# stripe/rainier

Hardware: NVIDIA H100
Metric: leapfrog_steps_x_chains_per_sec (higher is better)
Workload: dtype f64

## Files before the change

rainier_b200/csrc/rn_sampler.cuh:

```cuda
#ifndef RN_SAMPLER_CUH
#define RN_SAMPLER_CUH


#if RN_MASS_MAX >= 1
#define RN_TS_NMASS RN_N
#else
#define RN_TS_NMASS 0
#endif
#if RN_ENABLE_EHMC
#define RN_TS_NSNAP RN_N
#else
#define RN_TS_NSNAP 0
#endif
#ifndef RN_TS_RESTORE
#define RN_TS_RESTORE 0
#endif
#if RN_TS_RESTORE
#define RN_TS_NREST (2 * RN_N + 1)
#else
#define RN_TS_NREST 0
#endif
#define RN_TS_P 0
#define RN_TS_MASS (RN_N + 1)
#define RN_TS_SNAP (RN_TS_MASS + RN_TS_NMASS)
#define RN_TS_STAT (RN_TS_SNAP + RN_TS_NSNAP)
#define RN_TS_HOT (RN_TS_STAT + 5)
#define RN_TS_REST (RN_TS_HOT + 4)
#define RN_TS_DOUBLES (RN_TS_REST + RN_TS_NREST)
#define RN_TS_INTS 10
struct RnTs {
  double* d;
  int* i;
  unsigned bs;
};
#ifdef RN_HOST_EMULATION
static thread_local double rn_ts_mem_d[RN_TS_DOUBLES];
static thread_local int rn_ts_mem_i[RN_TS_INTS];
RN_DEVICE RnTs rn_ts_get() { return RnTs{rn_ts_mem_d, rn_ts_mem_i, 1u}; }
#define RN_STCS(ptr, v) (*(ptr) = (v))
#else
extern __shared__ double rn_ts_mem[];
RN_DEVICE RnTs rn_ts_get() {
  RnTs T;
#ifdef RN_BLOCK_DIM
  T.bs = RN_BLOCK_DIM;
#else
  T.bs = blockDim.x;
#endif
  T.d = rn_ts_mem + threadIdx.x;
  T.i = (int*)(rn_ts_mem + (size_t)RN_TS_DOUBLES * blockDim.x) + threadIdx.x;
  return T;
}
#define RN_STCS(ptr, v) __stcs((ptr), (v))
#endif
#define RN_TSD(slot) T.d[(unsigned)(slot) * T.bs]
#define RN_TSI(slot) T.i[(unsigned)(slot) * T.bs]
#ifndef RN_X_P_REGS
#define RN_X_P_REGS 1
#endif
#ifndef RN_X_NORMALS
#define RN_X_NORMALS 3
#endif
#define RN_Z(i) RN_TSD(RN_TS_P + (i))
#if RN_X_P_REGS
#define RN_P(i) s.p[i]
#else
#define RN_P(i) RN_TSD(RN_TS_P + (i))
#endif
#define RN_MASSD(i) RN_TSD(RN_TS_MASS + (i))
#define RN_SNAP_P(i) RN_TSD(RN_TS_SNAP + (i))
#define RN_ST_E_MEAN RN_TSD(RN_TS_STAT + 0)
#define RN_ST_E_RAW RN_TSD(RN_TS_STAT + 1)
#define RN_ST_TRANS2 RN_TSD(RN_TS_STAT + 2)
#define RN_ST_GRADS RN_TSD(RN_TS_STAT + 3)
#define RN_ST_STEPS RN_TSD(RN_TS_STAT + 4)
#define RN_ST_ITERS RN_TSI(0)
#define RN_ST_ACCEPTED RN_TSI(1)
#define RN_ST_E_N RN_TSI(2)
#define RN_ST_RING_I(r) RN_TSI(3 + (r))
#define RN_ST_RING_FULL(r) RN_TSI(6 + (r))
#define RN_TS_PREV_H RN_TSD(RN_TS_HOT + 2)
#define RN_TS_START_H RN_TSD(RN_TS_HOT + 3)
#define RN_REST_Q(i) RN_TSD(RN_TS_REST + (i))
#define RN_REST_G(i) RN_TSD(RN_TS_REST + RN_N + (i))
#define RN_REST_U RN_TSD(RN_TS_REST + 2 * RN_N)

struct RnIt {
  int grads, steps, err;
};

RN_DEVICE RnRng rn_rng_unpark(const RnTs& T) {
  RnRng r;
  r.seed = rn_d2ll(RN_TSD(RN_TS_HOT + 0));
  r.nng = RN_TSD(RN_TS_HOT + 1);
  r.have = RN_TSI(9);
  return r;
}
RN_DEVICE void rn_rng_park(const RnTs& T, const RnRng& r) {
  RN_TSD(RN_TS_HOT + 0) = rn_ll2d(r.seed);
  RN_TSD(RN_TS_HOT + 1) = r.nng;
  RN_TSI(9) = r.have;
}

RN_DEVICE void rn_ring_add(const RnArgs& A, int c, const RnTs& T, int which, double value) {
  int i = RN_ST_RING_I(which) + 1;
  if (i == A.stats_window) {
    RN_ST_RING_FULL(which) = 1;
    i = 0;
  }
  RN_ST_RING_I(which) = i;
  RN_STCS(&RN_AT(A.st_rings, which * A.stats_window + i, c), value);
}

struct RnPQ {
  double q[RN_N], g[RN_N];
  double U;
#if RN_X_P_REGS
  double p[RN_N];
#endif
};

RN_DEVICE double rn_velocity_i(const RnArgs& A, int c, const RnTs& T, const RnPQ& s, int kind, int i) {
  (void)s;
  (void)T;
  (void)A;
  (void)c;
#if RN_MASS_MAX >= 2
  if (kind == 2) {
    double y = 0.0;
    for (int j = 0; j < RN_N; j++) y += RN_P(j) * RN_AT(A.mass, i * RN_N + j, c);
    return y;
  }
#endif
#if RN_MASS_MAX >= 1
  if (kind == 1) return RN_P(i) * RN_MASSD(i);
#endif
  (void)kind;
  return RN_P(i);
}

RN_DEVICE double rn_energy(const RnArgs& A, int c, const RnTs& T, const RnPQ& s, int kind, double U) {
  double k = 0.0;
#if RN_MASS_MAX >= 2
  if (kind == 2) {
    for (int i = 0; i < RN_N; i++) k += (rn_velocity_i(A, c, T, s, 2, i) * RN_P(i));
    return U + k / 2.0;
  }
#endif
  RN_UNROLL
  for (int i = 0; i < RN_N; i++) k += (rn_velocity_i(A, c, T, s, kind, i) * RN_P(i));
  return U + k / 2.0;
}

RN_DEVICE double rn_log_accept(double deltaH) {
  if (deltaH != deltaH) return -RN_INF;
  return rn_jmin0(-deltaH);
}


RN_DEVICE void rn_update(const RnArgs& A, RnPQ& s, RnIt& S) {
  double dens;
  rn_density(s.q, dens, s.g, A.data, S.err);
  s.U = dens * -1;
  S.grads += 1;
}
RN_DEVICE void rn_full_ps(const RnTs& T, RnPQ& s, double stepSize, RnIt& S) {
  (void)T;
  S.grads += 1;
  RN_UNROLL
  for (int i = 0; i < RN_N; i++) RN_P(i) += stepSize * s.g[i];
}
RN_DEVICE void rn_new_qs(const RnArgs& A, int c, const RnTs& T, int kind, RnPQ& s, double stepSize) {
#if RN_MASS_MAX >= 2
  if (kind == 2) {
    for (int i = 0; i < RN_N; i++) s.q[i] += (stepSize * rn_velocity_i(A, c, T, s, 2, i));
    return;
  }
#endif
  RN_UNROLL
  for (int i = 0; i < RN_N; i++) s.q[i] += (stepSize * rn_velocity_i(A, c, T, s, kind, i));
}
RN_DEVICE void rn_leapfrog(const RnArgs& A, int c, const RnTs& T, int kind, RnPQ& s, int l, double stepSize, RnIt& S) {
  rn_full_ps(T, s, stepSize / 2.0, S);
  for (int i = 0;;) {
    rn_new_qs(A, c, T, kind, s, stepSize);
    rn_update(A, s, S);
    if (++i >= l) break;
    rn_full_ps(T, s, stepSize, S);
  }
  rn_full_ps(T, s, stepSize / 2.0, S);
}
RN_DEVICE void rn_take_steps(const RnArgs& A, int c, const RnTs& T, int kind, RnPQ& s, int l, double stepSize, RnIt& S) {
  rn_ring_add(A, c, T, 0, stepSize);
  rn_leapfrog(A, c, T, kind, s, l, stepSize, S);
  S.steps += l;
}

RN_DEVICE void rn_draw_normals(const RnTs& T, RnRng& rng) {
#if RN_X_NORMALS == 2
  for (int i = 0; i < RN_N; i++) RN_Z(i) = rn_normal(rng);
  return;
#endif
  int i0 = 0;
  if (rng.have) {
    rng.have = 0;
    RN_Z(0) = rng.nng;
    i0 = 1;
  }
  const int npairs = (RN_N - i0 + 1) / 2;
#ifndef RN_X_POLAR2
#define RN_X_POLAR2 1
#endif
#if RN_X_POLAR2
  for (int k = 0; k < npairs;) {
    double a1, a2, b1, b2;
    rn_i64 seed4, seed8;
    rn_polar_attempt2(rng, a1, a2, b1, b2, seed4, seed8);
    const double sa = a1 * a1 + a2 * a2, sb = b1 * b1 + b2 * b2;
    const bool oka = !(sa >= 1 || sa == 0);
    const int kb = k + (oka ? 1 : 0);
    const bool needb = kb < npairs;
    const bool okb = needb && !(sb >= 1 || sb == 0);
    if (oka) {
      RN_Z(i0 + 2 * k) = a1;
      RN_Z(i0 + 2 * k + 1) = a2;
    }
    if (okb) {
      RN_Z(i0 + 2 * kb) = b1;
      RN_Z(i0 + 2 * kb + 1) = b2;
    }
    rng.seed = needb ? seed8 : seed4;
    k = kb + (okb ? 1 : 0);
  }
#else
  for (int k = 0; k < npairs;) {
    double v1, v2;
    rn_polar_attempt(rng, v1, v2);
    const double s = v1 * v1 + v2 * v2;
    if (!(s >= 1 || s == 0)) {
      RN_Z(i0 + 2 * k) = v1;
      RN_Z(i0 + 2 * k + 1) = v2;
      k += 1;
    }
  }
#endif
#if RN_X_NORMALS == 4 && RN_X_SPEC && !defined(RN_FAST_MATH) && !(defined(RN_X_LIBM_PLAIN) && RN_X_LIBM_PLAIN)
#pragma unroll 1
  for (int k = 0; k < npairs; k += 2) {
    const int ia = i0 + 2 * k, ib = i0 + 2 * (k + 1 < npairs ? k + 1 : k);
    const double a1 = RN_Z(ia), a2 = RN_Z(ia + 1), b1 = RN_Z(ib), b2 = RN_Z(ib + 1);
    const double sa = a1 * a1 + a2 * a2, sb = b1 * b1 + b2 * b2;
    bool oka, okb;
    double la = rn_strict_log_try(sa, oka), lb = rn_strict_log_try(sb, okb);
    if (!(oka && okb)) {
      la = rn_strict_log_full(sa);
      lb = rn_strict_log_full(sb);
    }
    const double ma = rn_sqrt_nc(rn_div_nc(-2 * la, sa)), mb = rn_sqrt_nc(rn_div_nc(-2 * lb, sb));
    RN_Z(ia) = a1 * ma;
    if (ia + 1 < RN_N) {
      RN_Z(ia + 1) = a2 * ma;
    } else {
      rng.nng = a2 * ma;
      rng.have = 1;
    }
    RN_Z(ib) = b1 * mb;
    if (ib + 1 < RN_N) {
      RN_Z(ib + 1) = b2 * mb;
    } else {
      rng.nng = b2 * mb;
      rng.have = 1;
    }
  }
  return;
#endif
#if RN_X_NORMALS == 1
#pragma unroll 1
#elif RN_X_NORMALS == 3
#pragma unroll 2
#endif
  for (int k = 0; k < npairs; k++) {
    const int i = i0 + 2 * k;
    const double v1 = RN_Z(i), v2 = RN_Z(i + 1);
    const double s = v1 * v1 + v2 * v2;
    const double multiplier = rn_polar_multiplier(s);
    RN_Z(i) = v1 * multiplier;
    if (i + 1 < RN_N) {
      RN_Z(i + 1) = v2 * multiplier;
    } else {
      rng.nng = v2 * multiplier;
      rng.have = 1;
    }
  }
}

RN_DEVICE void rn_initialize_ps(const RnArgs& A, int c, const RnTs& T, RnPQ& s, int kind, RnRng& rng) {
  (void)A;
  (void)c;
  (void)kind;
  (void)s;
  rn_draw_normals(T, rng);
#if RN_X_P_REGS
  RN_UNROLL
  for (int i = 0; i < RN_N; i++) s.p[i] = RN_Z(i);
#endif
#if RN_MASS_MAX >= 2
  if (kind == 2) {
    int i = RN_N - 1;
    int m = ((i + 1) * (i + 2)) / 2 - 1;
    while (i >= 0) {
      int j = RN_N - 1;
      double dot = 0.0;
      while (j > i) {
        dot += RN_Z(j) * RN_AT(A.chol, m, c);
        j -= 1;
        m -= 1;
      }
      RN_Z(i) = (RN_Z(i) - dot) / RN_AT(A.chol, m, c);
      i -= 1;
      m -= 1;
    }
#if RN_X_P_REGS
    for (int k = 0; k < RN_N; k++) s.p[k] = RN_Z(k);
#endif
    return;
  }
#endif
#if RN_MASS_MAX >= 1
  if (kind == 1) {
    RN_UNROLL
    for (int i = 0; i < RN_N; i++) RN_P(i) = RN_P(i) / sqrt(RN_MASSD(i));
    return;
  }
#endif
}

RN_DEVICE void rn_load_mass(const RnArgs& A, int c, const RnTs& T, int kind) {
  (void)A;
  (void)c;
  (void)T;
  (void)kind;
#if RN_MASS_MAX >= 1
  if (kind == 1) {
    RN_UNROLL
    for (int i = 0; i < RN_N; i++) RN_MASSD(i) = RN_AT(A.mass, i, c);
  }
#endif
}

RN_DEVICE void rn_load_stats(const RnArgs& A, int c, const RnTs& T) {
  RN_ST_GRADS = rn_ll2d(A.st_grads[c]);
  RN_ST_STEPS = rn_ll2d(A.st_steps[c]);
  RN_ST_ITERS = A.st_iters[c];
  RN_ST_ACCEPTED = A.st_accepted[c];
  RN_ST_E_MEAN = RN_AT(A.st_energy, 0, c);
  RN_ST_E_RAW = RN_AT(A.st_energy, 1, c);
  RN_ST_TRANS2 = RN_AT(A.st_energy, 2, c);
  RN_ST_E_N = A.st_energy_n[c];
  for (int r = 0; r < 3; r++) {
    RN_ST_RING_I(r) = RN_AT(A.st_ring_i, r, c);
    RN_ST_RING_FULL(r) = RN_AT(A.st_ring_full, r, c);
  }
}
RN_DEVICE void rn_store_stats(const RnArgs& A, int c, const RnTs& T, int err) {
  A.st_grads[c] = rn_d2ll(RN_ST_GRADS);
  A.st_steps[c] = rn_d2ll(RN_ST_STEPS);
  A.st_iters[c] = RN_ST_ITERS;
  A.st_accepted[c] = RN_ST_ACCEPTED;
  if (err) A.st_err[c] |= err;
  RN_AT(A.st_energy, 0, c) = RN_ST_E_MEAN;
  RN_AT(A.st_energy, 1, c) = RN_ST_E_RAW;
  RN_AT(A.st_energy, 2, c) = RN_ST_TRANS2;
  A.st_energy_n[c] = RN_ST_E_N;
  for (int r = 0; r < 3; r++) {
    RN_AT(A.st_ring_i, r, c) = RN_ST_RING_I(r);
    RN_AT(A.st_ring_full, r, c) = RN_ST_RING_FULL(r);
  }
}
RN_DEVICE void rn_fold(const RnTs& T, RnIt& S) {
  RN_ST_GRADS = rn_ll2d(rn_d2ll(RN_ST_GRADS) + (rn_i64)S.grads);
  RN_ST_STEPS = rn_ll2d(rn_d2ll(RN_ST_STEPS) + (rn_i64)S.steps);
  S.grads = 0;
  S.steps = 0;
}

RN_GLOBAL void rn_k_init(const RnArgs A) {
  const int c = (int)(blockIdx.x * blockDim.x + threadIdx.x);
  if (c >= A.chains) return;
  const RnTs T = rn_ts_get();
  RnRng rng;
  rng.seed = A.rng_seed[c];
  rng.nng = A.rng_nng[c];
  rng.have = A.rng_have[c];
  rn_load_stats(A, c, T);
  RnIt S;
  S.grads = 0;
  S.steps = 0;
  S.err = 0;

  RnPQ s;
  rn_draw_normals(T, rng);
  RN_UNROLL
  for (int i = 0; i < RN_N; i++) s.q[i] = RN_Z(i);
  rn_update(A, s, S);
  double cq[RN_N], cg[RN_N];
  const double cU = s.U;
  RN_UNROLL
  for (int i = 0; i < RN_N; i++) {
    cq[i] = s.q[i];
    cg[i] = s.g[i];
  }
  rn_initialize_ps(A, c, T, s, 0, rng);
  RN_UNROLL
  for (int i = 0; i < RN_N; i++) RN_AT(A.params, i, c) = RN_P(i);

  double stepSize;
  if (A.step_tuner == 0) {
    const double H0 = rn_energy(A, c, T, s, 0, cU);
    stepSize = 1.0;
    double lap;
    rn_leapfrog(A, c, T, 0, s, 1, stepSize, S);
    lap = rn_log_accept(rn_energy(A, c, T, s, 0, s.U) - H0);
    const double exponent = (lap > -RN_LN2) ? 1.0 : -1.0;
    const double doubleOrHalf = (exponent > 0) ? 2.0 : 0.5;
#if RN_STEP_POOL
    int log2Step = 0;
#endif
    while (stepSize != 0.0 && (exponent * lap > -exponent * RN_LN2)) {
      stepSize *= doubleOrHalf;
#if RN_STEP_POOL
      log2Step += (exponent > 0) ? 1 : -1;
#endif
      RN_UNROLL
      for (int i = 0; i < RN_N; i++) {
        RN_P(i) = RN_AT(A.params, i, c);
        s.q[i] = cq[i];
        s.g[i] = cg[i];
      }
      s.U = cU;
      rn_leapfrog(A, c, T, 0, s, 1, stepSize, S);
      lap = rn_log_accept(rn_energy(A, c, T, s, 0, s.U) - H0);
    }
    rn_da_apply(stepSize, RN_AT(A.da, 1, c), RN_AT(A.da, 2, c), RN_AT(A.da, 3, c), RN_AT(A.da, 4, c), A.da_iter[c]);
#if RN_STEP_POOL
    rn_pool_add_initial_step(A.step_acc, log2Step);
#endif
  } else {
    stepSize = A.static_step;
  }
  RN_AT(A.da, 0, c) = stepSize;

  RN_UNROLL
  for (int i = 0; i < RN_N; i++) {
    RN_AT(A.params, RN_N + i, c) = cq[i];
    RN_AT(A.grad, i, c) = cg[i];
  }
  RN_AT(A.params, 2 * RN_N, c) = cU;
  A.rng_seed[c] = rng.seed;
  A.rng_nng[c] = rng.nng;
  A.rng_have[c] = rng.have;
  rn_fold(T, S);
  rn_store_stats(A, c, T, S.err);
}

enum { RN_P_IN_PARAMS = 0, RN_P_IN_REGS = 1, RN_P_IN_Z = 2 };
RN_DEVICE void rn_store_momentum(const RnArgs& A, int c, const RnTs& T, const RnPQ& s, int where) {
  (void)s;
  if (where == RN_P_IN_PARAMS) return;
  RN_UNROLL
  for (int i = 0; i < RN_N; i++) RN_AT(A.params, i, c) = where == RN_P_IN_REGS ? RN_P(i) : RN_Z(i);
}

template <int PHASE>
RN_DEVICE void rn_iterate(const RnArgs& A) {
  const int c = A.chain_begin + (int)(blockIdx.x * blockDim.x + threadIdx.x);
  if (c >= A.chain_end) return;
  const RnTs T = rn_ts_get();
  {
    RnRng rng;
    rng.seed = A.rng_seed[c];
    rng.nng = A.rng_nng[c];
    rng.have = A.rng_have[c];
    rn_rng_park(T, rng);
  }
  rn_load_stats(A, c, T);
  RnIt S;
  S.grads = 0;
  S.steps = 0;
  S.err = 0;
#if RN_MASS_MAX >= 1
  int kind = A.mass_kind;
#else
  constexpr int kind = 0;
#endif
  rn_load_mass(A, c, T, kind);

  double stepSize = RN_AT(A.da, 0, c);
  if (PHASE == 1 && A.step_tuner == 0) stepSize = rn_exp(RN_AT(A.da, 2, c));
  int win_size = A.win_size, win_i = A.win_i, win_j = A.win_j, est_samples = A.est_samples;
#if RN_ENABLE_EHMC
  int ring_i = 0, ring_full = 0;
  if (A.sampler == 1) {
    ring_i = A.ring_i[c];
    ring_full = A.ring_full[c];
  }
#endif
  bool havePrevH = false;

#ifndef RN_X_KEEP_STATE
#define RN_X_KEEP_STATE 1
#endif
#define RN_KEEP_P_LATE (RN_X_KEEP_STATE && RN_X_P_REGS)
#define RN_REST_ON_CHIP (RN_X_KEEP_STATE && RN_TS_RESTORE)
#if RN_REST_ON_CHIP
#define RN_X0(i) RN_REST_Q(i)
  int p_at = RN_P_IN_PARAMS;
#else
#define RN_X0(i) RN_AT(A.params, RN_N + (i), c)
#endif
  RnPQ s;
#if RN_X_KEEP_STATE
  RN_UNROLL
  for (int i = 0; i < RN_N; i++) {
    s.q[i] = RN_AT(A.params, RN_N + i, c);
    s.g[i] = RN_AT(A.grad, i, c);
  }
  s.U = RN_AT(A.params, 2 * RN_N, c);
#endif

  for (int it = 0; it < A.n_iter; it++) {
#if RN_X_KEEP_STATE
    const double cU = s.U;
#else
    const double cU = RN_AT(A.params, 2 * RN_N, c);
#endif
    if (!havePrevH) {
      RN_UNROLL
      for (int i = 0; i < RN_N; i++) RN_P(i) = RN_AT(A.params, i, c);
      RN_TS_PREV_H = rn_energy(A, c, T, s, kind, cU);
    }
    {
      RnRng rng = rn_rng_unpark(T);
      rn_initialize_ps(A, c, T, s, kind, rng);
      rn_rng_park(T, rng);
    }
#if RN_X_KEEP_STATE
    if (!(RN_KEEP_P_LATE && kind == 0)) {
      RN_UNROLL
      for (int i = 0; i < RN_N; i++) RN_AT(A.params, i, c) = RN_P(i);
    }
#else
    RN_UNROLL
    for (int i = 0; i < RN_N; i++) {
      RN_AT(A.params, i, c) = RN_P(i);
      s.q[i] = RN_AT(A.params, RN_N + i, c);
      s.g[i] = RN_AT(A.grad, i, c);
    }
#endif
    s.U = cU;
    RN_TS_START_H = rn_energy(A, c, T, s, kind, cU);
#if RN_REST_ON_CHIP
    RN_UNROLL
    for (int i = 0; i < RN_N; i++) {
      RN_REST_Q(i) = s.q[i];
      RN_REST_G(i) = s.g[i];
    }
    RN_REST_U = cU;
#endif
    const double usedStep = stepSize;

    if (A.sampler == 0) {
      rn_take_steps(A, c, T, kind, s, A.n_steps, stepSize, S);
    }
#if RN_ENABLE_EHMC
    else {
      bool count = false;
      if (PHASE == 0 && !ring_full) count = true;
      else if (PHASE == 0) {
        RnRng rng = rn_rng_unpark(T);
        count = rn_uniform(rng) < A.p_count;
        rn_rng_park(T, rng);
      }
      if (count) {
        RnPQ snap;
        int l = 0;
        for (;;) {
          double out = 0.0;
          RN_UNROLL
          for (int i = 0; i < RN_N; i++) out += (s.q[i] - RN_X0(i)) * RN_P(i);
          const bool uturn = (out != out) ? true : (out < 0);
          if (uturn || !(l < A.max_steps)) break;
          l += 1;
          rn_take_steps(A, c, T, kind, s, 1, stepSize, S);
          if (l == A.min_steps) {
            snap = s;
#if !(RN_X_P_REGS)
            RN_UNROLL
            for (int i = 0; i < RN_N; i++) RN_SNAP_P(i) = RN_P(i);
#endif
          }
        }
        if (l < A.min_steps) {
          rn_take_steps(A, c, T, kind, s, A.min_steps - l, stepSize, S);
        } else {
          s = snap;
#if !(RN_X_P_REGS)
          RN_UNROLL
          for (int i = 0; i < RN_N; i++) RN_P(i) = RN_SNAP_P(i);
#endif
        }
        ring_i += 1;
        if (ring_i == A.buf_size) ring_full = 1;
        ring_i = ring_i % A.buf_size;
        RN_AT(A.ring, ring_i, c) = (double)l;
      } else {
        RnRng rng = rn_rng_unpark(T);
        const int idx = ring_full ? rn_rng_int(rng, A.buf_size) : rn_rng_int(rng, ring_i + 1);
        rn_rng_park(T, rng);
        const int nsteps = rn_d2i(RN_AT(A.ring, idx, c));
        rn_take_steps(A, c, T, kind, s, nsteps, stepSize, S);
      }
    }
#endif

    const double endH = rn_energy(A, c, T, s, kind, s.U);
    const double startH = RN_TS_START_H;
    const double deltaH = endH - startH;
    const double a = rn_log_accept(deltaH);
    bool accept;
    {
      RnRng rng = rn_rng_unpark(T);
      accept = a > rn_log(rn_uniform(rng));
      rn_rng_park(T, rng);
    }
    double eH;
    if (accept) {
#if RN_REST_ON_CHIP
      p_at = RN_P_IN_REGS;
#else
      RN_UNROLL
      for (int i = 0; i < RN_N; i++) {
        RN_AT(A.params, i, c) = RN_P(i);
        RN_AT(A.params, RN_N + i, c) = s.q[i];
        RN_AT(A.grad, i, c) = s.g[i];
      }
      RN_AT(A.params, 2 * RN_N, c) = s.U;
#endif
      eH = endH;
      RN_ST_ACCEPTED += 1;
    } else {
#if RN_REST_ON_CHIP
      RN_UNROLL
      for (int i = 0; i < RN_N; i++) {
        s.q[i] = RN_REST_Q(i);
        s.g[i] = RN_REST_G(i);
      }
      s.U = RN_REST_U;
      p_at = (RN_KEEP_P_LATE && kind == 0) ? RN_P_IN_Z : RN_P_IN_PARAMS;
#else
      RN_UNROLL
      for (int i = 0; i < RN_N; i++) s.q[i] = RN_AT(A.params, RN_N + i, c);
#if RN_X_KEEP_STATE
      RN_UNROLL
      for (int i = 0; i < RN_N; i++) s.g[i] = RN_AT(A.grad, i, c);
      s.U = RN_AT(A.params, 2 * RN_N, c);
      if (RN_KEEP_P_LATE && kind == 0) {
        RN_UNROLL
        for (int i = 0; i < RN_N; i++) RN_AT(A.params, i, c) = RN_Z(i);
      }
#endif
#endif
      eH = startH;
    }
    {
      const int e_n = RN_ST_E_N + 1;
      RN_ST_E_N = e_n;
      double e_mean = RN_ST_E_MEAN;
      const double oldDiff = eH - e_mean;
      e_mean += (oldDiff / (double)e_n);
      RN_ST_E_MEAN = e_mean;
      const double newDiff = eH - e_mean;
      RN_ST_E_RAW += oldDiff * newDiff;
      const double d = eH - RN_TS_PREV_H;
      RN_ST_TRANS2 += d * d;
    }
    RN_TS_PREV_H = eH;
    havePrevH = true;
    RN_ST_ITERS += 1;
    rn_ring_add(A, c, T, 1, rn_exp(a));
    rn_ring_add(A, c, T, 2, (double)S.grads);

    if (A.trace) {
      double* tr = A.trace + (size_t)it * 4 * (size_t)A.chains;
      tr[0 * (size_t)A.chains + c] = a;
      tr[1 * (size_t)A.chains + c] = accept ? 1.0 : 0.0;
      tr[2 * (size_t)A.chains + c] = usedStep;
      tr[3 * (size_t)A.chains + c] = (double)S.steps;
    }
    rn_fold(T, S);

    if (PHASE == 0) {
#if RN_STEP_POOL
      if (A.step_tuner == 0) rn_pool_add(A.step_acc + it, rn_pool_quantise(rn_exp(a)));
#else
      if (A.step_tuner == 0) {
        const double newAcceptanceProb = rn_exp(a);
        const int daIter = A.da_iter[c] + 1;
        A.da_iter[c] = daIter;
        const double avgErrorMultiplier = 1.0 / ((double)daIter + 10);
        const double stepSizeMultiplier = rn_pow((double)daIter, -0.75);
        const double avgError = ((1.0 - avgErrorMultiplier) * RN_AT(A.da, 3, c) + (avgErrorMultiplier * (A.delta - newAcceptanceProb)));
        RN_AT(A.da, 3, c) = avgError;
        const double logStepSize = (RN_AT(A.da, 4, c) - (avgError * sqrt((double)daIter) / 0.05));
        RN_AT(A.da, 1, c) = logStepSize;
        RN_AT(A.da, 2, c) = (stepSizeMultiplier * logStepSize + (1.0 - stepSizeMultiplier) * RN_AT(A.da, 2, c));
        stepSize = rn_exp(logStepSize);
      }
#endif
#if RN_MASS_MAX >= 1
      if (A.mass_tuner == 1 || A.mass_tuner == 2) {
        win_j += 1;
        if (A.adaptation == 1) {
          if (RN_IN_WINDOW(A, win_j)) {
            win_i += 1;
#if RN_MASS_POOL
            double oldDiff[RN_N], newDiff[RN_N];
            RN_UNROLL
            for (int i = 0; i < RN_N; i++) newDiff[i] = rn_variance_update(A, c, i, s.q[i], win_i, oldDiff[i]);
            for (int j = 0; j < RN_N; j++)
              for (int k = 0; k < RN_N; k++) RN_AT(A.est_cov, j * RN_N + k, c) += newDiff[j] * oldDiff[k];
#else
            RN_UNROLL
            for (int i = 0; i < RN_N; i++) {
              double oldDiff;
              rn_variance_update(A, c, i, s.q[i], win_i, oldDiff);
            }
#endif
            if (win_i == win_size) {
              win_i = 0;
              win_size = rn_d2i(win_size * A.win_expansion);
            }
          }
        } else if (RN_IN_WINDOW(A, win_j)) {
          win_i += 1;
          est_samples += 1;
#if RN_MASS_MAX >= 2
          double oldDiff[RN_N], newDiff[RN_N];
          RN_UNROLL
          for (int i = 0; i < RN_N; i++) newDiff[i] = rn_variance_update(A, c, i, s.q[i], est_samples, oldDiff[i]);
#else
          RN_UNROLL
          for (int i = 0; i < RN_N; i++) {
            double oldDiff;
            rn_variance_update(A, c, i, s.q[i], est_samples, oldDiff);
          }
#endif
#if RN_MASS_MAX >= 2
          if (A.mass_tuner == 2) {
            for (int j = 0; j < RN_N; j++)
              for (int k = 0; k < RN_N; k++) RN_AT(A.est_cov, j * RN_N + k, c) += newDiff[j] * oldDiff[k];
          }
#endif
          if (win_i == win_size) {
            win_i = 0;
            win_size = rn_d2i(win_size * A.win_expansion);
            havePrevH = false;
#if RN_REST_ON_CHIP
            rn_store_momentum(A, c, T, s, p_at);
            p_at = RN_P_IN_PARAMS;
#endif
            if (A.mass_tuner == 1) {
              kind = 1;
              RN_UNROLL
              for (int i = 0; i < RN_N; i++) {
                const double v = RN_AT(A.est_raw, i, c) / (double)est_samples;
                if (v == 0.0) S.err |= 2;
                RN_MASSD(i) = v;
                RN_AT(A.mass, i, c) = v;
                RN_AT(A.est_mean, i, c) = 0.0;
                RN_AT(A.est_raw, i, c) = 0.0;
              }
            }
#if RN_MASS_MAX >= 2
            else {
              kind = 2;
              const double z = (double)(est_samples - 1);
              for (int i = 0; i < RN_N * RN_N; i++) {
                const double v = RN_AT(A.est_cov, i, c) / z;
                if (v == 0.0) S.err |= 2;
                RN_AT(A.mass, i, c) = v;
                RN_AT(A.est_cov, i, c) = 0.0;
              }
              for (int i = 0; i < RN_N; i++) {
                RN_AT(A.est_mean, i, c) = 0.0;
                RN_AT(A.est_raw, i, c) = 0.0;
              }
              double lower[(RN_N * (RN_N + 1)) / 2];
              rn_cholesky_upper(A, c, lower, 1);
            }
#endif
#if !RN_STEP_POOL
            if (A.step_tuner == 0)
              stepSize = rn_da_reset(RN_AT(A.da, 1, c), RN_AT(A.da, 2, c), RN_AT(A.da, 3, c), RN_AT(A.da, 4, c), A.da_iter[c]);
#endif
          }
        }
      }
#endif
    } else if (A.samples) {
      double* out = A.samples + (size_t)it * RN_N * (size_t)A.chains;
      RN_UNROLL
      for (int i = 0; i < RN_N; i++) RN_STCS(&out[(size_t)i * (size_t)A.chains + c], s.q[i]);
    }
  }

#if RN_REST_ON_CHIP
  rn_store_momentum(A, c, T, s, p_at);
  RN_UNROLL
  for (int i = 0; i < RN_N; i++) {
    RN_AT(A.params, RN_N + i, c) = s.q[i];
    RN_AT(A.grad, i, c) = s.g[i];
  }
  RN_AT(A.params, 2 * RN_N, c) = s.U;
#endif
  if (PHASE == 0) RN_AT(A.da, 0, c) = stepSize;
#if RN_ENABLE_EHMC
  if (A.sampler == 1) {
    A.ring_i[c] = ring_i;
    A.ring_full[c] = ring_full;
  }
#endif
  {
    const RnRng rng = rn_rng_unpark(T);
    A.rng_seed[c] = rng.seed;
    A.rng_nng[c] = rng.nng;
    A.rng_have[c] = rng.have;
  }
  rn_store_stats(A, c, T, S.err);
}
RN_GLOBAL void rn_k_warmup(const RnArgs A) { rn_iterate<0>(A); }
RN_GLOBAL void rn_k_iter(const RnArgs A) { rn_iterate<1>(A); }
#define RN_K_WARMUP rn_k_warmup

RN_GLOBAL void rn_k_density(const double* RN_RESTRICT qin, double* RN_RESTRICT out, const double* data, int* err,
                            int chains) {
  const int c = (int)(blockIdx.x * blockDim.x + threadIdx.x);
  if (c >= chains) return;
  double q[RN_N], g[RN_N], dens;
  RN_UNROLL
  for (int i = 0; i < RN_N; i++) q[i] = qin[(size_t)i * chains + c];
  int e = 0;
  rn_density(q, dens, g, data, e);
  out[c] = dens;
  RN_UNROLL
  for (int i = 0; i < RN_N; i++) out[(size_t)(i + 1) * chains + c] = g[i];
#ifdef RN_HOST_EMULATION
  if (e) *err |= e;
#else
  if (e) atomicOr(err, e);
#endif
}

#endif
```

Before: 29.03 billion.

## Interleave next iteration's polar normal draws into the leapfrog loop

Splits the polar normal sampler into begin/trip/finish pieces. For the plain HMC sampler, it draws the acceptance uniform up front, then runs one rejection trip for the next iteration's momenta inside each leapfrog step, between the position update and the gradient evaluation. The aim is to hide RNG and rejection-loop latency behind gradient work and shorten the serial draw phase between iterations. This reorders RNG consumption, so the random stream differs from before, and it adds register pressure and branching inside the inner loop.

```diff
diff --git a/rainier_b200/csrc/rn_sampler.cuh b/rainier_b200/csrc/rn_sampler.cuh
--- a/rainier_b200/csrc/rn_sampler.cuh
+++ b/rainier_b200/csrc/rn_sampler.cuh
@@ -157,93 +157,38 @@
   return rn_jmin0(-deltaH);
 }
 
-
-RN_DEVICE void rn_update(const RnArgs& A, RnPQ& s, RnIt& S) {
-  double dens;
-  rn_density(s.q, dens, s.g, A.data, S.err);
-  s.U = dens * -1;
-  S.grads += 1;
-}
-RN_DEVICE void rn_full_ps(const RnTs& T, RnPQ& s, double stepSize, RnIt& S) {
-  (void)T;
-  S.grads += 1;
-  RN_UNROLL
-  for (int i = 0; i < RN_N; i++) RN_P(i) += stepSize * s.g[i];
-}
-RN_DEVICE void rn_new_qs(const RnArgs& A, int c, const RnTs& T, int kind, RnPQ& s, double stepSize) {
-#if RN_MASS_MAX >= 2
-  if (kind == 2) {
-    for (int i = 0; i < RN_N; i++) s.q[i] += (stepSize * rn_velocity_i(A, c, T, s, 2, i));
-    return;
-  }
-#endif
-  RN_UNROLL
-  for (int i = 0; i < RN_N; i++) s.q[i] += (stepSize * rn_velocity_i(A, c, T, s, kind, i));
-}
-RN_DEVICE void rn_leapfrog(const RnArgs& A, int c, const RnTs& T, int kind, RnPQ& s, int l, double stepSize, RnIt& S) {
-  rn_full_ps(T, s, stepSize / 2.0, S);
-  for (int i = 0;;) {
-    rn_new_qs(A, c, T, kind, s, stepSize);
-    rn_update(A, s, S);
-    if (++i >= l) break;
-    rn_full_ps(T, s, stepSize, S);
-  }
-  rn_full_ps(T, s, stepSize / 2.0, S);
-}
-RN_DEVICE void rn_take_steps(const RnArgs& A, int c, const RnTs& T, int kind, RnPQ& s, int l, double stepSize, RnIt& S) {
-  rn_ring_add(A, c, T, 0, stepSize);
-  rn_leapfrog(A, c, T, kind, s, l, stepSize, S);
-  S.steps += l;
-}
-
-RN_DEVICE void rn_draw_normals(const RnTs& T, RnRng& rng) {
-#if RN_X_NORMALS == 2
-  for (int i = 0; i < RN_N; i++) RN_Z(i) = rn_normal(rng);
-  return;
-#endif
-  int i0 = 0;
+RN_DEVICE int rn_polar_begin(const RnTs& T, RnRng& rng) {
   if (rng.have) {
     rng.have = 0;
     RN_Z(0) = rng.nng;
-    i0 = 1;
-  }
+    return 1;
+  }
+  return 0;
+}
+RN_DEVICE void rn_polar_trip(const RnTs& T, RnRng& rng, int& j) {
+  double a1, a2, b1, b2;
+  rn_i64 seed4, seed8;
+  rn_polar_attempt2(rng, a1, a2, b1, b2, seed4, seed8);
+  const double sa = a1 * a1 + a2 * a2, sb = b1 * b1 + b2 * b2;
+  const bool needa = j < RN_N;
+  const bool oka = needa && !(sa >= 1 || sa == 0);
+  const int jb = j + (oka ? 2 : 0);
+  const bool needb = jb < RN_N;
+  const bool okb = needb && !(sb >= 1 || sb == 0);
+  if (oka) {
+    RN_Z(j) = a1;
+    RN_Z(j + 1) = a2;
+  }
+  if (okb) {
+    RN_Z(jb) = b1;
+    RN_Z(jb + 1) = b2;
+  }
+  rng.seed = needb ? seed8 : (needa ? seed4 : rng.seed);
+  j = jb + (okb ? 2 : 0);
+}
+RN_DEVICE void rn_polar_finish(const RnTs& T, RnRng& rng, int j) {
+  const int i0 = j & 1;
   const int npairs = (RN_N - i0 + 1) / 2;
-#ifndef RN_X_POLAR2
-#define RN_X_POLAR2 1
-#endif
-#if RN_X_POLAR2
-  for (int k = 0; k < npairs;) {
-    double a1, a2, b1, b2;
-    rn_i64 seed4, seed8;
-    rn_polar_attempt2(rng, a1, a2, b1, b2, seed4, seed8);
-    const double sa = a1 * a1 + a2 * a2, sb = b1 * b1 + b2 * b2;
-    const bool oka = !(sa >= 1 || sa == 0);
-    const int kb = k + (oka ? 1 : 0);
-    const bool needb = kb < npairs;
-    const bool okb = needb && !(sb >= 1 || sb == 0);
-    if (oka) {
-      RN_Z(i0 + 2 * k) = a1;
-      RN_Z(i0 + 2 * k + 1) = a2;
-    }
-    if (okb) {
-      RN_Z(i0 + 2 * kb) = b1;
-      RN_Z(i0 + 2 * kb + 1) = b2;
-    }
-    rng.seed = needb ? seed8 : seed4;
-    k = kb + (okb ? 1 : 0);
-  }
-#else
-  for (int k = 0; k < npairs;) {
-    double v1, v2;
-    rn_polar_attempt(rng, v1, v2);
-    const double s = v1 * v1 + v2 * v2;
-    if (!(s >= 1 || s == 0)) {
-      RN_Z(i0 + 2 * k) = v1;
-      RN_Z(i0 + 2 * k + 1) = v2;
-      k += 1;
-    }
-  }
-#endif
 #if RN_X_NORMALS == 4 && RN_X_SPEC && !defined(RN_FAST_MATH) && !(defined(RN_X_LIBM_PLAIN) && RN_X_LIBM_PLAIN)
 #pragma unroll 1
   for (int k = 0; k < npairs; k += 2) {
@@ -293,13 +238,66 @@
     }
   }
 }
-
-RN_DEVICE void rn_initialize_ps(const RnArgs& A, int c, const RnTs& T, RnPQ& s, int kind, RnRng& rng) {
+RN_DEVICE void rn_draw_normals(const RnTs& T, RnRng& rng) {
+  int j = rn_polar_begin(T, rng);
+  while (j < RN_N) rn_polar_trip(T, rng, j);
+  rn_polar_finish(T, rng, j);
+}
+
+RN_DEVICE void rn_update(const RnArgs& A, RnPQ& s, RnIt& S) {
+  double dens;
+  rn_density(s.q, dens, s.g, A.data, S.err);
+  s.U = dens * -1;
+  S.grads += 1;
+}
+RN_DEVICE void rn_full_ps(const RnTs& T, RnPQ& s, double stepSize, RnIt& S) {
+  (void)T;
+  S.grads += 1;
+  RN_UNROLL
+  for (int i = 0; i < RN_N; i++) RN_P(i) += stepSize * s.g[i];
+}
+RN_DEVICE void rn_new_qs(const RnArgs& A, int c, const RnTs& T, int kind, RnPQ& s, double stepSize) {
+#if RN_MASS_MAX >= 2
+  if (kind == 2) {
+    for (int i = 0; i < RN_N; i++) s.q[i] += (stepSize * rn_velocity_i(A, c, T, s, 2, i));
+    return;
+  }
+#endif
+  RN_UNROLL
+  for (int i = 0; i < RN_N; i++) s.q[i] += (stepSize * rn_velocity_i(A, c, T, s, kind, i));
+}
+RN_DEVICE void rn_leapfrog(const RnArgs& A, int c, const RnTs& T, int kind, RnPQ& s, int l, double stepSize, RnIt& S,
+                           int* draw = nullptr) {
+  rn_full_ps(T, s, stepSize / 2.0, S);
+  for (int i = 0;;) {
+    rn_new_qs(A, c, T, kind, s, stepSize);
+    if (draw) {
+      RnRng rng = rn_rng_unpark(T);
+      rn_polar_trip(T, rng, *draw);
+      rn_rng_park(T, rng);
+    }
+    rn_update(A, s, S);
+    if (++i >= l) break;
+    rn_full_ps(T, s, stepSize, S);
+  }
+  rn_full_ps(T, s, stepSize / 2.0, S);
+}
+RN_DEVICE void rn_take_steps(const RnArgs& A, int c, const RnTs& T, int kind, RnPQ& s, int l, double stepSize, RnIt& S,
+                             int* draw = nullptr) {
+  rn_ring_add(A, c, T, 0, stepSize);
+  rn_leapfrog(A, c, T, kind, s, l, stepSize, S, draw);
+  S.steps += l;
+}
+
+RN_DEVICE void rn_initialize_ps(const RnArgs& A, int c, const RnTs& T, RnPQ& s, int kind, RnRng& rng, int drawn = -1) {
   (void)A;
   (void)c;
   (void)kind;
   (void)s;
-  rn_draw_normals(T, rng);
+  if (drawn >= 0)
+    rn_polar_finish(T, rng, drawn);
+  else
+    rn_draw_normals(T, rng);
 #if RN_X_P_REGS
   RN_UNROLL
   for (int i = 0; i < RN_N; i++) s.p[i] = RN_Z(i);
@@ -527,6 +525,10 @@
   }
   s.U = RN_AT(A.params, 2 * RN_N, c);
 #endif
+#define RN_DRAW_AHEAD (RN_REST_ON_CHIP && RN_KEEP_P_LATE)
+  bool ahead = false;
+  int draw = RN_N;
+  double logu = 0.0;
 
   for (int it = 0; it < A.n_iter; it++) {
 #if RN_X_KEEP_STATE
@@ -541,7 +543,7 @@
     }
     {
       RnRng rng = rn_rng_unpark(T);
-      rn_initialize_ps(A, c, T, s, kind, rng);
+      rn_initialize_ps(A, c, T, s, kind, rng, ahead ? draw : -1);
       rn_rng_park(T, rng);
     }
 #if RN_X_KEEP_STATE
@@ -568,9 +570,33 @@
     RN_REST_U = cU;
 #endif
     const double usedStep = stepSize;
+#if RN_DRAW_AHEAD
+    {
+      bool closes = false;
+#if RN_MASS_MAX >= 1
+      if (PHASE == 0 && (A.mass_tuner == 1 || A.mass_tuner == 2)) closes = RN_IN_WINDOW(A, win_j + 1) && win_i + 1 == win_size;
+#endif
+      ahead = A.sampler == 0 && it + 1 < A.n_iter && !closes;
+      RnRng rng = rn_rng_unpark(T), next = rng;
+      const double lu = rn_log(rn_uniform(next));
+      if (A.sampler == 0) {
+        rng = next;
+        logu = lu;
+      }
+      draw = RN_N;
+      if (ahead) draw = rn_polar_begin(T, rng);
+      rn_rng_park(T, rng);
+    }
+#endif
 
     if (A.sampler == 0) {
-      rn_take_steps(A, c, T, kind, s, A.n_steps, stepSize, S);
+      rn_take_steps(A, c, T, kind, s, A.n_steps, stepSize, S, RN_DRAW_AHEAD ? &draw : nullptr);
+      if (draw < RN_N) {
+        RnRng rng = rn_rng_unpark(T);
+        do rn_polar_trip(T, rng, draw);
+        while (draw < RN_N);
+        rn_rng_park(T, rng);
+      }
     }
 #if RN_ENABLE_EHMC
     else {
@@ -627,12 +653,12 @@
     const double startH = RN_TS_START_H;
     const double deltaH = endH - startH;
     const double a = rn_log_accept(deltaH);
-    bool accept;
-    {
+    if (!(RN_DRAW_AHEAD && A.sampler == 0)) {
       RnRng rng = rn_rng_unpark(T);
-      accept = a > rn_log(rn_uniform(rng));
+      logu = rn_log(rn_uniform(rng));
       rn_rng_park(T, rng);
     }
+    const bool accept = a > logu;
     double eH;
     if (accept) {
 #if RN_REST_ON_CHIP
```

Result: faster. 29.63 billion, median of 6 (+2.1%).
